# 0xEigenLabs/eigen-zeth

Hardware: AMD Instinct MI355X
Metric: goldilocks_ntt_field_elems_per_s (higher is better)
Workload: dtype u64; 1 GPU; forward NTT, natural order in/out, 2^24 rows x 64 columns per GPU (column-major u64), BASELINE configs[3] shape on one GPU; logn=24, cols_per_gpu=64, cols_total=64

## Files before the change

### eigen_zeth_amd/csrc/ntt.hip

```cpp
#include <hip/hip_runtime.h>

#include <cstring>
#include <string>

#include "ctx.hpp"
#include "wave_xchg.hpp"
#include "gl_asm.hpp"
#include "gl_limb.hpp"

#define ZP_LDG(p) __builtin_nontemporal_load(p)
#define ZP_STG(p, v) __builtin_nontemporal_store(v, p)

namespace {

typedef __attribute__((ext_vector_type(4))) int zp_i32x4;

struct PassArgs {
    const u64 *in;
    u64 *out;
    u64 in_cs, out_cs;
    u64 in_valid;
    const u64 *twl, *twh;
    const u64 *tws;
    const u64 *tw1;
    const u64 *itab;
    const u64 *csl, *csh;
    u64 scale;
    int logn, logPprev, lb, cslb;
    int j0inv;
    int logPin;
    int flags;
    int ncols;
};

__device__ __forceinline__ constexpr int brev(int x, int bits) {
    int r = 0;
    for (int i = 0; i < bits; i++) r |= ((x >> i) & 1) << (bits - 1 - i);
    return r;
}
__device__ __forceinline__ constexpr int slot_of(int o, int j, int pos, int A) {
    return ((o >> pos) << (pos + A)) | (j << pos) | (o & ((1 << pos) - 1));
}

template <int A1, int A2, int A3, int LOGT>
struct Geo {
    static constexpr int L = A1 + A2 + A3;
    static constexpr int R = 1 << L;
    static constexpr int T = 1 << LOGT;
    static constexpr int LT = LOGT;
    static constexpr int NT = (R * T) / 16;
    static constexpr int J = 1 + (A2 > 0 ? 1 : 0) + (A3 > 0 ? 1 : 0);
    static constexpr int POS1 = L - A1;
    static constexpr int POS2 = L - A1 - A2;
    static constexpr int AJ = (J == 1) ? A1 : (J == 2 ? A2 : A3);
    __device__ static __forceinline__ int kof(int sigma) {
        int k = (sigma >> POS1) & ((1 << A1) - 1);
        if (A2 > 0) k |= ((sigma >> POS2) & ((1 << A2) - 1)) << A1;
        if (A3 > 0) k |= (sigma & ((1 << A3) - 1)) << (A1 + A2);
        return k;
    }
    __device__ static __forceinline__ int sigma_of_k(int k) {
        int s = (k & ((1 << A1) - 1)) << POS1;
        if (A2 > 0) s |= ((k >> A1) & ((1 << A2) - 1)) << POS2;
        if (A3 > 0) s |= (k >> (A1 + A2)) & ((1 << A3) - 1);
        return s;
    }
    __device__ static __forceinline__ int lpos(int sigma, int t) {
        int s2 = sigma;
        if constexpr (LOGT < 4 && A3 > 0) {
            constexpr int GB = 5 - LOGT;
            s2 ^= ((sigma >> POS2) & ((1 << GB) - 1)) ^ (((sigma >> (POS1 + LOGT)) & ((1 << (A1 - LOGT)) - 1)) << 1);
        }
        return (s2 << LOGT) + (t ^ (kof(sigma) & (T - 1)));
    }
};

__device__ __forceinline__ u64 tw_lookup(const u64 *lo, const u64 *hi, int lb, u64 e) {
    u64 a = lo[e & ((1ULL << lb) - 1)];
    u64 b = hi[e >> lb];
    return gl_mul(a, b);
}

__device__ __forceinline__ u64 mul_c16(int e, u64 d) {
    switch (e) {
        case 0: return d;
        case 1: return gl_shl12<1>(d);
        case 2: return gl_shl12<2>(d);
        case 3: return gl_shl12<3>(d);
        case 4: return gl_shl12<4>(d);
        case 5: return gl_shl12<5>(d);
        case 6: return gl_shl12<6>(d);
        default: return gl_shl12<7>(d);
    }
}
template <int A>
__device__ __forceinline__ void dif_shift(u64 *v) {
    static_assert(A >= 2 && A <= 4, "radix 4, 8 or 16");
#pragma unroll
    for (int s = 0; s < A; s++) {
        const int half = 1 << (A - 1 - s);
#pragma unroll
        for (int t = 0; t < (1 << (A - 1)); t += 2) {
            const int i0 = (t / half) * 2 * half + (t % half), i1 = ((t + 1) / half) * 2 * half + ((t + 1) % half);
            gl_bfly2(v[i0], v[i0 + half], v[i1], v[i1 + half]);
            v[i0 + half] = mul_c16((t % half) * (8 / half), v[i0 + half]);
            v[i1 + half] = mul_c16(((t + 1) % half) * (8 / half), v[i1 + half]);
        }
    }
}

__device__ __forceinline__ void lds_barrier() {
    __builtin_amdgcn_fence(__ATOMIC_RELEASE, "workgroup", "local");
    __builtin_amdgcn_s_barrier();
    __builtin_amdgcn_fence(__ATOMIC_ACQUIRE, "workgroup", "local");
}

template <typename G, int ANEXT, int POSNEXT>
__device__ __forceinline__ void exchange_read(u64 *v, const u64 *lds, int tid) {
    constexpr int GN = 16 >> ANEXT;
#pragma unroll
    for (int g = 0; g < GN; g++) {
        const int gamma = g * G::NT + tid;
        const int t = gamma & (G::T - 1), o = gamma >> G::LT;
#pragma unroll
        for (int j = 0; j < (1 << ANEXT); j++)
            v[g * (1 << ANEXT) + j] = lds[G::lpos(slot_of(o, j, POSNEXT, ANEXT), t)];
    }
}

template <typename G, int A, int POS, int ANEXT, int POSNEXT, int TWSH>
__device__ __forceinline__ void exchange2(u64 *v, u64 *lds, const u64 *twr, int j0inv, int tid) {
    constexpr int GR = 16 >> A;
#pragma unroll
    for (int g = 0; g < GR; g++) {
        const int gamma = g * G::NT + tid;
        const int t = gamma & (G::T - 1), o = gamma >> G::LT;
        const int rho = o & ((1 << POS) - 1);
        {
            const int kj1 = (j0inv * brev(1, A)) & ((1 << A) - 1);
            v[g * (1 << A) + 1] = gl_mul1(v[g * (1 << A) + 1], twr[(kj1 * rho) << TWSH]);
        }
#pragma unroll
        for (int p = 2; p < (1 << A); p += 2) {
            const int kja = (j0inv * brev(p, A)) & ((1 << A) - 1), kjb = (j0inv * brev(p + 1, A)) & ((1 << A) - 1);
            gl_mul2(v[g * (1 << A) + p], twr[(kja * rho) << TWSH], v[g * (1 << A) + p + 1], twr[(kjb * rho) << TWSH]);
        }
#pragma unroll
        for (int p = 0; p < (1 << A); p++) {
            const int kj = (j0inv * brev(p, A)) & ((1 << A) - 1);
            lds[G::lpos(slot_of(o, kj, POS, A), t)] = v[g * (1 << A) + p];
        }
    }
    lds_barrier();
    exchange_read<G, ANEXT, POSNEXT>(v, lds, tid);
}

template <int E>
__device__ __forceinline__ gl_l4 mul_c16_l4(const gl_l4 &d) { return gl_l4_mul_c16<E>(d); }
__device__ __forceinline__ gl_l4 mul_c16_l4(int e, const gl_l4 &d) {
    switch (e) {
        case 0: return d;
        case 1: return gl_l4_mul_c16<1>(d);
        case 2: return gl_l4_mul_c16<2>(d);
        case 3: return gl_l4_mul_c16<3>(d);
        case 4: return gl_l4_mul_c16<4>(d);
        case 5: return gl_l4_mul_c16<5>(d);
        case 6: return gl_l4_mul_c16<6>(d);
        default: return gl_l4_mul_c16<7>(d);
    }
}
template <int A>
__device__ __forceinline__ void dif_levels_l4(gl_l4 *x) {
    static_assert(A >= 2 && A <= 4, "radix 4, 8 or 16");
#pragma unroll
    for (int s = 0; s < A; s++) {
        const int half = 1 << (A - 1 - s);
#pragma unroll
        for (int t = 0; t < (1 << (A - 1)); t++) {
            const int i0 = (t / half) * 2 * half + (t % half);
            const gl_l4 a = x[i0], b = x[i0 + half];
            x[i0] = gl_l4_add(a, b);
            x[i0 + half] = mul_c16_l4((t % half) * (8 / half), gl_l4_sub(a, b));
        }
    }
}
template <int A>
__device__ __forceinline__ void dif_shift_l4(const u64 *v, gl_l4 *x) {
#pragma unroll
    for (int i = 0; i < (1 << A); i++) x[i] = gl_l4_from(v[i]);
    dif_levels_l4<A>(x);
}
__device__ __forceinline__ gl_w4 w4_load(const gl_w4 *p) {
    const zp_i32x4 a = *(const zp_i32x4 *)p->lo, b = *(const zp_i32x4 *)p->hi;
    gl_w4 w;
    w.lo[0] = a.x; w.lo[1] = a.y; w.lo[2] = a.z; w.lo[3] = a.w;
    w.hi[0] = b.x; w.hi[1] = b.y; w.hi[2] = b.z; w.hi[3] = b.w;
    return w;
}
__device__ __forceinline__ void w4_store(gl_w4 *p, const u64 w0, const u64 w1, const u64 w2, const u64 w3) {
    i32 l[4], h[4];
    gl_l4_balance(w0, l[0], h[0]);
    gl_l4_balance(w1, l[1], h[1]);
    gl_l4_balance(w2, l[2], h[2]);
    gl_l4_balance(w3, l[3], h[3]);
    zp_i32x4 a = {l[0], l[1], l[2], l[3]}, b = {h[0], h[1], h[2], h[3]};
    *(zp_i32x4 *)p->lo = a;
    *(zp_i32x4 *)p->hi = b;
}
template <typename G, int A, int POS, int ANEXT, int POSNEXT>
__device__ __forceinline__ void exchange2_l4(const gl_l4 *x, u64 *v, u64 *lds, const gl_w4 *twr4, int j0inv, int tid) {
    constexpr int GR = 16 >> A;
#pragma unroll
    for (int g = 0; g < GR; g++) {
        const int gamma = g * G::NT + tid;
        const int t = gamma & (G::T - 1), o = gamma >> G::LT;
        const int rho = o & ((1 << POS) - 1);
#pragma unroll
        for (int p = 0; p < (1 << A); p++) {
            const int kj = (j0inv * brev(p, A)) & ((1 << A) - 1);
            const u64 y = p == 0 ? gl_l4_canon(x[g * (1 << A)]) : gl_l4_mul(x[g * (1 << A) + p], w4_load(twr4 + kj * rho));
            lds[G::lpos(slot_of(o, kj, POS, A), t)] = y;
        }
    }
    lds_barrier();
    exchange_read<G, ANEXT, POSNEXT>(v, lds, tid);
}

template <typename G>
__device__ __forceinline__ void table_copy_out(u64 *v, const u64 *lds, const u64 *twb, u64 *blk, int tid) {
    constexpr int L = G::L, NT = G::NT;
#pragma unroll
    for (int i = 0; i < 16; i++) v[i] = twb[i * NT + tid];
    lds_barrier();
#pragma unroll
    for (int i = 0; i < 16; i += 2) {
        const int ia = i * NT + tid, ib = (i + 1) * NT + tid;
        u64 xa = lds[G::lpos(G::sigma_of_k(ia & ((1 << L) - 1)), ia >> L)];
        u64 xb = lds[G::lpos(G::sigma_of_k(ib & ((1 << L) - 1)), ib >> L)];
        gl_mul2(xa, v[i], xb, v[i + 1]);
        ZP_STG(&blk[ia], xa);
        ZP_STG(&blk[ib], xb);
    }
}

template <int A1, int A2, int A3, int LOGT, bool TRANSPOSE, bool PADDED, int MODE, bool BIG = false, bool LIMB = false>
__global__ void __launch_bounds__((1 << (A1 + A2 + A3 + LOGT)) / 16, LIMB ? 3 : 4)
ntt_pass2_kernel(PassArgs a, int tiles_per_wg) {
    using G = Geo<A1, A2, A3, LOGT>;
    constexpr int L = G::L, R = G::R, T = G::T, NT = G::NT, AJ = G::AJ;
    constexpr int GRJ = 16 >> AJ;
    constexpr int R2 = 1 << (A2 + A3);
    constexpr bool HAS_TAB = !TRANSPOSE && MODE >= 1;
    constexpr bool TWR_LDS = L <= 10;
    constexpr int TPL = (R + NT - 1) / NT;
    extern __shared__ __attribute__((aligned(16))) u64 lds[];
    constexpr int REC = LIMB ? 4 : 1;
    u64 *tab = lds + R * T;
    u64 *twr1 = tab + (HAS_TAB ? R * REC : 0);
    u64 *twr2 = twr1 + R * REC;
    constexpr bool TW1 = TRANSPOSE && MODE == 3;
    constexpr bool CAN_IN = !TRANSPOSE && MODE == 0 && L <= 9;
    u64 *itl = twr2 + (TWR_LDS ? R2 * REC : 0);
    const bool in_tab = CAN_IN && a.itab != nullptr;
    static_assert(!LIMB || (TWR_LDS && (TW1 || !TRANSPOSE)), "limb form: LDS twiddle copies, no per-lane twiddle chain");
    u64 col = blockIdx.y, wg_lin = blockIdx.x;
    if constexpr (TW1) {
        const u64 x = blockIdx.x & 7u, j = blockIdx.x >> 3;
        col = j % (u64)a.ncols;
        wg_lin = (j / (u64)a.ncols) * 8 + x;
    }
    const int logNR = a.logn - L;
    const int logP = a.logPprev;
    const u64 N = 1ULL << a.logn;
    const u64 *src = a.in + col * a.in_cs;
    u64 *dst = a.out + col * a.out_cs;
    u64 v[16], vn[16];
    constexpr int NTW = TW1 ? 1 : TRANSPOSE ? (GRJ + 2) : (MODE == 2 ? TPL + 1 : TPL);
    u64 twl_c[NTW], twh_c[NTW], twl_n[NTW], twh_n[NTW];

    constexpr bool small_n = !BIG;
    auto fetch_tile = [&](u64 *r, u64 *tl, u64 *th, u64 u0, int tid) {
        constexpr int GR = 16 >> A1;
        const u64 valid_rows = a.in_valid >> logNR;
#pragma unroll
        for (int g = 0; g < GR; g++) {
            const int gamma = g * NT + tid;
            const int t = gamma & (T - 1), o = gamma >> LOGT;
            const u32 slot0 = (u32)slot_of(o, 0, G::POS1, A1);
            const u32 lane_bytes = (((u32)slot0 << logNR) + (u32)t) << 3;
            const u64 lane_el = ((u64)slot0 << logNR) + (u64)t;
#pragma unroll
            for (int j = 0; j < (1 << A1); j++) {
                const u64 *rowp = src + (((u64)j << G::POS1) << logNR) + u0;
                const u64 *ptr;
                if constexpr (small_n) ptr = (const u64 *)((const char *)rowp + lane_bytes);
                else ptr = rowp + lane_el;
                u64 val;
                if constexpr (PADDED) val = (u64)(slot0 + ((u32)j << G::POS1)) < valid_rows ? (LOGT < 4 ? *ptr : ZP_LDG(ptr)) : 0ULL;
                else val = LOGT < 4 ? *ptr : ZP_LDG(ptr);
                r[g * (1 << A1) + j] = val;
            }
        }
        const u64 lm = (1ULL << a.lb) - 1;
        if constexpr (TW1) {
            (void)tl; (void)th; (void)lm;
        } else if constexpr (TRANSPOSE) {
            const int t = tid & (T - 1);
            const u64 u = u0 + t;
            const int jr = a.j0inv & ((1 << AJ) - 1);
            u64 e[NTW];
#pragma unroll
            for (int g = 0; g < GRJ; g++) e[g] = u * (u64)G::kof(((g * NT + tid) >> LOGT) << AJ);
            e[GRJ] = ((u << (L - AJ)) * (u64)jr) & (N - 1);
            e[GRJ + 1] = (N - ((u << L) & (N - 1))) & (N - 1);
#pragma unroll
            for (int i = 0; i < NTW; i++) { tl[i] = a.twl[e[i] & lm]; th[i] = a.twh[e[i] >> a.lb]; }
        } else {
            if constexpr (MODE == 1) {
                if (a.flags & 1) {
                    const u64 e0 = (u0 >> logP) << logP;
#pragma unroll
                    for (int j = 0; j < TPL; j++) {
                        const u64 e = e0 * (u64)((tid + j * NT) & (R - 1));
                        tl[j] = a.twl[e & lm];
                        th[j] = a.twh[e >> a.lb];
                    }
                }
            }
            if constexpr (CAN_IN) {
                if (in_tab) {
                    const u64 *row = a.itab + ((u0 >> a.logPin) << L);
#pragma unroll
                    for (int j = 0; j < TPL; j++) tl[j] = row[(tid + j * NT) & (R - 1)];
                }
            }
            if constexpr (MODE == 2) {
                const u64 c = (u0 + (tid & (T - 1))) & ((1ULL << logP) - 1);
                tl[TPL] = a.csl[c & ((1ULL << a.cslb) - 1)];
                th[TPL] = a.csh[c >> a.cslb];
            }
        }
    };

    u64 wg = wg_lin;
    if constexpr (LOGT < 4 && !TW1) {
        if ((gridDim.x & 7u) == 0) wg = (u64)(blockIdx.x & 7u) * (gridDim.x >> 3) + (blockIdx.x >> 3);
    }
    const u64 tile0 = wg * tiles_per_wg;
    fetch_tile(v, twl_c, twh_c, tile0 << LOGT, threadIdx.x);
    const bool out_tab = HAS_TAB && (MODE == 2 || (a.flags & 3) != 0);
    const bool tile_tab = HAS_TAB && (a.flags & 1) != 0;
    {
        const int tid0 = threadIdx.x;
        if constexpr (LIMB) {
            for (int e = tid0; e < R; e += NT) {
                const int rot = (a.j0inv * (R / 8)) & (R - 1);
                w4_store((gl_w4 *)twr1 + e, a.tws[e << (12 - L)], a.tws[((e + rot) & (R - 1)) << (12 - L)],
                         a.tws[((e + 2 * rot) & (R - 1)) << (12 - L)], a.tws[((e + 3 * rot) & (R - 1)) << (12 - L)]);
            }
            if constexpr (G::J >= 3) {
                constexpr int L2 = A2 + A3;
                for (int e = tid0; e < R2; e += NT) {
                    const int rot = (a.j0inv * (R2 / 8)) & (R2 - 1);
                    w4_store((gl_w4 *)twr2 + e, a.tws[e << (12 - L2)], a.tws[((e + rot) & (R2 - 1)) << (12 - L2)],
                             a.tws[((e + 2 * rot) & (R2 - 1)) << (12 - L2)], a.tws[((e + 3 * rot) & (R2 - 1)) << (12 - L2)]);
                }
            }
        } else if constexpr (TWR_LDS) {
            if (tid0 < R) twr1[tid0] = a.tws[tid0 << (12 - L)];
            if constexpr (G::J >= 3) {
                if (tid0 < R2) twr2[tid0] = a.tws[tid0 << (12 - (A2 + A3))];
            }
        }
        if constexpr (HAS_TAB) {
            if (out_tab && !tile_tab) {
#pragma unroll
                for (int j = 0; j < TPL; j++)
                    if (tid0 + j * NT < R) {
                        u64 w = (a.flags & 2) ? a.scale : 1;
                        if constexpr (MODE == 2) {
                            const u64 ek = (u64)(tid0 + j * NT) << logP;
                            const u64 ck = gl_mul(a.csl[ek & ((1ULL << a.cslb) - 1)], a.csh[ek >> a.cslb]);
                            w = (a.flags & 2) ? gl_mul(w, ck) : ck;
                        }
                        if constexpr (LIMB) w4_store((gl_w4 *)tab + tid0 + j * NT, w, gl_shl12<2>(w), gl_shl12<4>(w), gl_shl12<6>(w));
                        else tab[tid0 + j * NT] = w;
                    }
            }
        }
        if constexpr (CAN_IN) {
            if (in_tab) {
#pragma unroll
                for (int j = 0; j < TPL; j++)
                    if (tid0 + j * NT < R) itl[tid0 + j * NT] = twl_c[j];
            }
        }
    }
    lds_barrier();
    __builtin_amdgcn_s_waitcnt(0x0F70);
#pragma clang loop unroll(disable)
    for (int it = 0; it < tiles_per_wg; it++) {
        const u64 u0 = (tile0 + it) << LOGT;
        const bool more = it + 1 < tiles_per_wg;
        int tid = threadIdx.x;
        asm volatile("" : "+v"(tid));
        if (more) fetch_tile(vn, twl_n, twh_n, u0 + T, tid);

        const u64 s = TRANSPOSE ? 0 : (u0 >> logP);
        if constexpr (HAS_TAB) {
            if (tile_tab) {
#pragma unroll
                for (int j = 0; j < TPL; j++)
                    if (tid + j * NT < R) {
                        const u64 w = gl_mul(twl_c[j], twh_c[j]);
                        if constexpr (LIMB) w4_store((gl_w4 *)tab + tid + j * NT, w, gl_shl12<2>(w), gl_shl12<4>(w), gl_shl12<6>(w));
                        else tab[tid + j * NT] = w;
                    }
            }
        }
        if constexpr (CAN_IN) {
            if (in_tab) {
#pragma unroll
                for (int g = 0; g < (16 >> A1); g++) {
                    const int slot0 = slot_of((g * NT + tid) >> LOGT, 0, G::POS1, A1);
#pragma unroll
                    for (int j = 0; j < (1 << A1); j += 2)
                        gl_mul2(v[g * (1 << A1) + j], itl[(j << G::POS1) + slot0], v[g * (1 << A1) + j + 1], itl[((j + 1) << G::POS1) + slot0]);
                }
            }
        }
        gl_l4 x[LIMB ? 16 : 1];
        if constexpr (LIMB) {
#pragma unroll
            for (int g = 0; g < (16 >> A1); g++) dif_shift_l4<A1>(v + g * (1 << A1), x + g * (1 << A1));
            exchange2_l4<G, A1, G::POS1, A2, G::POS2>(x, v, lds, (const gl_w4 *)twr1, a.j0inv, tid);
#pragma unroll
            for (int g = 0; g < (16 >> A2); g++) dif_shift_l4<A2>(v + g * (1 << A2), x + g * (1 << A2));
            if constexpr (G::J >= 3) {
                exchange2_l4<G, A2, G::POS2, A3, 0>(x, v, lds, (const gl_w4 *)twr2, a.j0inv, tid);
#pragma unroll
                for (int g = 0; g < (16 >> A3); g++) dif_shift_l4<A3>(v + g * (1 << A3), x + g * (1 << A3));
            }
        } else {
#pragma unroll
        for (int g = 0; g < (16 >> A1); g++) dif_shift<A1>(v + g * (1 << A1));
        exchange2<G, A1, G::POS1, A2, G::POS2, TWR_LDS ? 0 : 12 - L>(v, lds, TWR_LDS ? twr1 : a.tws, a.j0inv, tid);
#pragma unroll
        for (int g = 0; g < (16 >> A2); g++) dif_shift<A2>(v + g * (1 << A2));
        if constexpr (G::J >= 3) {
            exchange2<G, A2, G::POS2, A3, 0, TWR_LDS ? 0 : 12 - (A2 + A3)>(v, lds, TWR_LDS ? twr2 : a.tws, a.j0inv, tid);
#pragma unroll
            for (int g = 0; g < (16 >> A3); g++) dif_shift<A3>(v + g * (1 << A3));
        }
        }
#pragma unroll
        for (int g = 0; g < GRJ; g++) {
            const int gamma = g * NT + tid;
            const int t = gamma & (T - 1), o = gamma >> LOGT;
            const int klow = G::kof(o << AJ);
            if constexpr (TW1) {
                const int jr = a.j0inv & ((1 << AJ) - 1);
#pragma unroll
                for (int i = 0; i < (1 << AJ); i++) {
                    const int kj = (jr * i) & ((1 << AJ) - 1);
                    if constexpr (LIMB) lds[G::lpos(slot_of(o, kj, 0, AJ), t)] = gl_l4_canon(x[g * (1 << AJ) + brev(i, AJ)]);
                    else lds[G::lpos(slot_of(o, kj, 0, AJ), t)] = v[g * (1 << AJ) + brev(i, AJ)];
                }
            } else if constexpr (TRANSPOSE) {
                const int jr = a.j0inv & ((1 << AJ) - 1);
                u64 w = gl_mul(twl_c[g], twh_c[g]);
                const u64 hj = gl_mul(twl_c[GRJ], twh_c[GRJ]);
                const u64 hjd = gl_mul(hj, gl_mul(twl_c[GRJ + 1], twh_c[GRJ + 1]));
#pragma unroll
                for (int i = 0; i < (1 << AJ); i++) {
                    const int p = brev(i, AJ);
                    const int kj = (jr * i) & ((1 << AJ) - 1);
                    u64 x = v[g * (1 << AJ) + p];
                    if (i + 1 < (1 << AJ)) {
                        const bool wrap = ((jr * (i + 1)) >> AJ) != ((jr * i) >> AJ);
                        u64 wn = w;
                        gl_mul2(x, w, wn, wrap ? hjd : hj);
                        w = wn;
                    } else {
                        x = gl_mul1(x, w);
                    }
                    lds[G::lpos(slot_of(o, kj, 0, AJ), t)] = x;
                }
            } else {
                u64 *const sbase = dst + (s << (logP + L)) + (u0 & ((1ULL << logP) - 1));
                const u32 lane_sb = (((u32)klow << logP) + (u32)t) << 3;
                const u64 lane_se = ((u64)klow << logP) + (u64)t;
                u64 cw = 1;
                if constexpr (MODE == 2) cw = gl_mul(twl_c[TPL], twh_c[TPL]);
#pragma unroll
                for (int p = 0; p < (1 << AJ); p += 2) {
                    const int kja = (a.j0inv * brev(p, AJ)) & ((1 << AJ) - 1), kjb = (a.j0inv * brev(p + 1, AJ)) & ((1 << AJ) - 1);
                    const int ka = klow + (kja << (L - AJ)), kb = klow + (kjb << (L - AJ));
                    u64 xa, xb;
                    if constexpr (LIMB) {
                        if (out_tab) {
                            xa = gl_l4_mul(x[g * (1 << AJ) + p], w4_load((const gl_w4 *)tab + ka));
                            xb = gl_l4_mul(x[g * (1 << AJ) + p + 1], w4_load((const gl_w4 *)tab + kb));
                        } else {
                            xa = gl_l4_canon(x[g * (1 << AJ) + p]);
                            xb = gl_l4_canon(x[g * (1 << AJ) + p + 1]);
                        }
                    } else {
                        xa = v[g * (1 << AJ) + p];
                        xb = v[g * (1 << AJ) + p + 1];
                        if (out_tab) gl_mul2(xa, tab[ka], xb, tab[kb]);
                    }
                    if constexpr (MODE == 2) gl_mul2(xa, cw, xb, cw);
                    u64 *const ua = sbase + ((u64)(kja << (L - AJ)) << logP), *const ub = sbase + ((u64)(kjb << (L - AJ)) << logP);
                    u64 *pa, *pb;
                    if constexpr (small_n) { pa = (u64 *)((char *)ua + lane_sb); pb = (u64 *)((char *)ub + lane_sb); }
                    else { pa = ua + lane_se; pb = ub + lane_se; }
                    if constexpr (LOGT < 4) {
                        *pa = xa;
                        *pb = xb;
                    } else {
                        ZP_STG(pa, xa);
                        ZP_STG(pb, xb);
                    }
                }
            }
        }
        if constexpr (TW1) {
            table_copy_out<G>(v, lds, a.tw1 + (u0 << L), dst + (u0 << L), tid);
        } else if constexpr (TRANSPOSE) {
            lds_barrier();
            u64 *blk = dst + (u0 << L);
#pragma unroll
            for (int i = 0; i < 16; i++) {
                const int idx = i * NT + tid;
                const int t2 = idx >> L, k = idx & ((1 << L) - 1);
                ZP_STG(&blk[idx], lds[G::lpos(G::sigma_of_k(k), t2)]);
            }
        }
        if (more) {
            if constexpr (CAN_IN) {
                if (in_tab) {
#pragma unroll
                    for (int j = 0; j < TPL; j++)
                        if (tid + j * NT < R) itl[tid + j * NT] = twl_n[j];
                }
            }
            lds_barrier();
#pragma unroll
            for (int i = 0; i < 16; i++) v[i] = vn[i];
#pragma unroll
            for (int i = 0; i < NTW; i++) { twl_c[i] = twl_n[i]; twh_c[i] = twh_n[i]; }
        }
    }
}

struct SeamArgs {
    const u64 *in;
    u64 *out;
    u64 *coef;
    const u64 *tws_i, *tws_f;
    const u64 *tw1;
    const u64 *csl, *csh;
    u64 scale;
    int logn, cslb, j0inv_i, j0inv_f, ncols;
};
__global__ void __launch_bounds__(256, 4) lde_seam_kernel(SeamArgs a, int tiles_per_wg) {
    using G = Geo<4, 4, 0, 4>;
    constexpr int L = 8, R = 256, T = 16, LOGT = 4;
    extern __shared__ __attribute__((aligned(16))) u64 lds[];
    u64 *tab = lds + R * T;
    u64 *twr_i = tab + R;
    u64 *twr_f = twr_i + R;
    const u64 x8 = blockIdx.x & 7u, jj = blockIdx.x >> 3;
    const u64 col = jj % (u64)a.ncols, wg = (jj / (u64)a.ncols) * 8 + x8;
    const int logNR = a.logn - L;
    const u64 N = 1ULL << a.logn;
    const u64 *src = a.in + col * N;
    u64 *dst = a.out + col * (2 * N);
    u64 *cdst = a.coef ? a.coef + col * N : nullptr;
    u64 v[16];
    u64 cw_c[2];
    auto fetch_tile = [&](u64 *r, u64 *cwr, u64 u0, int tid) {
        const int t = tid & (T - 1), o = tid >> LOGT;
        const u32 slot0 = (u32)slot_of(o, 0, G::POS1, 4);
        const u32 lane_bytes = (((u32)slot0 << logNR) + (u32)t) << 3;
#pragma unroll
        for (int j = 0; j < 16; j++) {
            const u64 *rowp = src + (((u64)j << G::POS1) << logNR) + u0;
            r[j] = ZP_LDG((const u64 *)((const char *)rowp + lane_bytes));
        }
        const u64 c = u0 + (u64)t;
        cwr[0] = a.csl[c & ((1ULL << a.cslb) - 1)];
        cwr[1] = a.csh[c >> a.cslb];
    };
    const u64 tile0 = wg * tiles_per_wg;
    {
        const int tid0 = threadIdx.x;
        twr_i[tid0] = a.tws_i[tid0 << (12 - L)];
        twr_f[tid0] = a.tws_f[tid0 << (12 - L)];
        const u64 ek = (u64)tid0 << logNR;
        tab[tid0] = gl_mul(a.scale, gl_mul(a.csl[ek & ((1ULL << a.cslb) - 1)], a.csh[ek >> a.cslb]));
    }
    lds_barrier();
#pragma clang loop unroll(disable)
    for (int it = 0; it < tiles_per_wg; it++) {
        const u64 u0 = (tile0 + it) << LOGT;
        int tid = threadIdx.x;
        asm volatile("" : "+v"(tid));
        fetch_tile(v, cw_c, u0, tid);
        const int t = tid & (T - 1), o = tid >> LOGT;
        dif_shift<4>(v);
        exchange2<G, 4, G::POS1, 4, G::POS2, 0>(v, lds, twr_i, a.j0inv_i, tid);
        dif_shift<4>(v);
        const u64 cw = gl_mul(cw_c[0], cw_c[1]);
        lds_barrier();
#pragma unroll
        for (int p = 0; p < 16; p += 2) {
            const int kja = (a.j0inv_i * brev(p, 4)) & 15, kjb = (a.j0inv_i * brev(p + 1, 4)) & 15;
            const int ka = o + (kja << 4), kb = o + (kjb << 4);
            u64 xa = v[p], xb = v[p + 1];
            gl_mul2(xa, tab[ka], xb, tab[kb]);
            gl_mul2(xa, cw, xb, cw);
            if (cdst) {
                ZP_STG((u64 *)((char *)(cdst + ((u64)ka << logNR) + u0) + (t << 3)), xa);
                ZP_STG((u64 *)((char *)(cdst + ((u64)kb << logNR) + u0) + (t << 3)), xb);
            }
            lds[(((ka & 1) << 7) + (ka >> 1)) * T + t] = xa;
            lds[(((kb & 1) << 7) + (kb >> 1)) * T + t] = xb;
        }
        lds_barrier();
        u64 f1[8];
#pragma unroll
        for (int j = 0; j < 8; j++) {
            v[j] = lds[((j << 4) + o) * T + t];
            f1[j] = lds[(128 + (j << 4) + o) * T + t];
        }
        lds_barrier();
#pragma unroll 1
        for (int par = 0; par < 2; par++) {
            if (par) {
#pragma unroll
                for (int j = 0; j < 8; j++) v[j] = f1[j];
            }
#pragma unroll
            for (int j = 1; j < 8; j++) v[8 + j] = mul_c16(j, v[j]);
            v[8] = v[0];
            dif_shift<3>(v);
            dif_shift<3>(v + 8);
            exchange2<G, 4, G::POS1, 4, G::POS2, 0>(v, lds, twr_f, a.j0inv_f, tid);
            dif_shift<4>(v);
            {
                const int jr = a.j0inv_f & 15;
#pragma unroll
                for (int i = 0; i < 16; i++) {
                    const int kj = (jr * i) & 15;
                    lds[G::lpos(slot_of(o, kj, 0, 4), t)] = v[brev(i, 4)];
                }
            }
            const u64 u0f = ((u64)par << logNR) + u0;
            table_copy_out<G>(v, lds, a.tw1 + (u0f << L), dst + (u0f << L), tid);
            lds_barrier();
        }
    }
}

struct SmallArgs {
    const u64 *in;
    u64 *out;
    u64 in_cs, out_cs, in_valid;
    const u64 *tws;
    const u64 *csl, *csh;
    u64 scale;
    int logn, cslb, flags;
};

template <int LH>
__device__ __forceinline__ u64 wave_stage(u64 x, int lane, const u64 *tws) {
    const u64 y = lane_xor<LH>(x);
    const int i = lane & ((1 << LH) - 1);
    if (!((lane >> LH) & 1)) return gl_add(x, y);
    const u64 d = gl_sub(y, x);
    return i ? gl_mul(d, tws[(u64)i << (12 - (LH + 1))]) : d;
}

template <bool WAVE>
__global__ void __launch_bounds__(256) ntt_small_kernel(SmallArgs a) {
    extern __shared__ __attribute__((aligned(16))) u64 lds[];
    const int tid = threadIdx.x;
    const int n = 1 << a.logn;
    const u64 *src = a.in + (u64)blockIdx.x * a.in_cs;
    u64 *dst = a.out + (u64)blockIdx.x * a.out_cs;
    for (int i = tid; i < n; i += 256) lds[i] = (u64)i < a.in_valid ? src[i] : 0ULL;
    __syncthreads();
    const int lds_stages = WAVE ? (a.logn > 6 ? a.logn - 6 : 0) : a.logn;
    for (int s = 0; s < lds_stages; s++) {
        const int lh = a.logn - 1 - s;
        const int half = 1 << lh;
        for (int b = tid; b < (n >> 1); b += 256) {
            const int i = b & (half - 1);
            const int i0 = ((b >> lh) << (lh + 1)) + i, i1 = i0 + half;
            u64 x = lds[i0], y = lds[i1];
            lds[i0] = gl_add(x, y);
            u64 d = gl_sub(x, y);
            lds[i1] = i ? gl_mul(d, a.tws[(u64)i << (12 - (lh + 1))]) : d;
        }
        __syncthreads();
    }
    if constexpr (WAVE) {
        const int lane = tid & 63;
        for (int base = (tid >> 6) << 6; base < n; base += 256) {
            u64 x = base + lane < n ? lds[base + lane] : 0ULL;
            const int top = a.logn < 6 ? a.logn : 6;
            if (top >= 6) x = wave_stage<5>(x, lane, a.tws);
            if (top >= 5) x = wave_stage<4>(x, lane, a.tws);
            if (top >= 4) x = wave_stage<3>(x, lane, a.tws);
            if (top >= 3) x = wave_stage<2>(x, lane, a.tws);
            if (top >= 2) x = wave_stage<1>(x, lane, a.tws);
            if (top >= 1) x = wave_stage<0>(x, lane, a.tws);
            const int i = base + lane;
            if (i < n) {
                const int k = brev(i, a.logn);
                if (a.flags & 2) x = gl_mul(x, a.scale);
                if (a.flags & 4) x = gl_mul(x, tw_lookup(a.csl, a.csh, a.cslb, (u64)k));
                dst[k] = x;
            }
        }
        return;
    }
    for (int i = tid; i < n; i += 256) {
        const int k = brev(i, a.logn);
        u64 x = lds[i];
        if (a.flags & 2) x = gl_mul(x, a.scale);
        if (a.flags & 4) x = gl_mul(x, tw_lookup(a.csl, a.csh, a.cslb, (u64)k));
        dst[k] = x;
    }
}

__global__ void __launch_bounds__(256) coset_scale_kernel(const u64 *in, u64 *out, u64 n, const u64 *lo,
                                                         const u64 *hi, int lb) {
    const u64 col = blockIdx.y;
    const u64 i = ((u64)blockIdx.x * 256 + threadIdx.x);
    if (i < n) out[col * n + i] = gl_mul(in[col * n + i], tw_lookup(lo, hi, lb, i));
}

__global__ void __launch_bounds__(256) twiddle_rows_kernel(u64 *rows, int logn_row, u64 total, u64 row0, u64 nmask,
                                                           const u64 *lo, const u64 *hi, int lb) {
    const u64 i = (u64)blockIdx.x * 256 + threadIdx.x;
    if (i >= total) return;
    const u64 r = i >> logn_row, k = i & ((1ULL << logn_row) - 1);
    const u64 e = ((row0 + r) * k) & nmask;
    rows[i] = gl_mul(rows[i], tw_lookup(lo, hi, lb, e));
}

__global__ void __launch_bounds__(256) tw1_fill_kernel(u64 *out, int logn, int L, const u64 *lo, const u64 *hi, int lb) {
    const u64 i = (u64)blockIdx.x * 256 + threadIdx.x;
    if (i >> logn) return;
    const u64 u = i >> L, k = i & ((1ULL << L) - 1);
    out[i] = tw_lookup(lo, hi, lb, (u * k) & ((1ULL << logn) - 1));
}

__global__ void __launch_bounds__(256) itab_fill_kernel(u64 *out, u64 total, int logn, int L, int logPp, u64 pre, const u64 *lo, const u64 *hi, int lb) {
    const u64 i = (u64)blockIdx.x * 256 + threadIdx.x;
    if (i >= total) return;
    const u64 k = i >> L, r = i & ((1ULL << L) - 1);
    out[i] = gl_mul(pre, tw_lookup(lo, hi, lb, ((k * r) << logPp) & ((1ULL << logn) - 1)));
}

using PassKernel = void (*)(PassArgs, int);

template <int A1, int A2, int A3, int LOGT, bool BIG>
PassKernel pick_pass_kernel(bool transpose, bool table, bool padded, int mode, bool limb) {
    constexpr bool CAN_TABLE = !BIG && A3 == 0, CAN_LIMB = !BIG && A1 + A2 + A3 <= 8;
    if constexpr (CAN_TABLE) {
        if (table && limb) return padded ? ntt_pass2_kernel<A1, A2, A3, LOGT, true, true, 3, false, CAN_LIMB> : ntt_pass2_kernel<A1, A2, A3, LOGT, true, false, 3, false, CAN_LIMB>;
        if (table) return padded ? ntt_pass2_kernel<A1, A2, A3, LOGT, true, true, 3, false> : ntt_pass2_kernel<A1, A2, A3, LOGT, true, false, 3, false>;
    }
    if (transpose) return padded ? ntt_pass2_kernel<A1, A2, A3, LOGT, true, true, 1, BIG> : ntt_pass2_kernel<A1, A2, A3, LOGT, true, false, 1, BIG>;
    if (limb) return mode == 2 ? ntt_pass2_kernel<A1, A2, A3, LOGT, false, false, 2, BIG, CAN_LIMB>
                   : mode == 1 ? ntt_pass2_kernel<A1, A2, A3, LOGT, false, false, 1, BIG, CAN_LIMB>
                               : ntt_pass2_kernel<A1, A2, A3, LOGT, false, false, 0, BIG, CAN_LIMB>;
    return mode == 2 ? ntt_pass2_kernel<A1, A2, A3, LOGT, false, false, 2, BIG>
         : mode == 1 ? ntt_pass2_kernel<A1, A2, A3, LOGT, false, false, 1, BIG>
                     : ntt_pass2_kernel<A1, A2, A3, LOGT, false, false, 0, BIG>;
}

template <int A1, int A2, int A3, int LOGT, bool BIG = false>
int32_t launch_pass2(zp_ctx *ctx, PassArgs a, bool transpose, int W) {
    using G = Geo<A1, A2, A3, LOGT>;
    const u64 tiles = (1ULL << (a.logn - G::L)) >> LOGT;
    int tpw = ctx->tune_tpw;
    while (tpw > 1 && (tiles % tpw != 0 || tiles / tpw * (u64)W < (u64)ctx->num_cu * 4)) tpw >>= 1;
    dim3 grid((unsigned)(tiles / tpw), (unsigned)W), block(G::NT);
    const bool table = !BIG && A3 == 0 && transpose && a.tw1 && (grid.x & 7u) == 0;
    const int mode = transpose ? 0 : (a.flags & 4) ? 2 : (a.flags & 11) ? 1 : 0;
    const bool limb = !BIG && G::L <= 8 && ctx->tune_ntt_limb != 0 && (!transpose || table);
    const size_t rec = limb ? 4 : 1;
    const size_t shmem = ((size_t)G::R * G::T + (mode >= 1 ? G::R * rec : 0) + (G::L <= 10 ? (G::R + (1 << (A2 + A3))) * rec : 0) + (a.itab ? G::R : 0)) * sizeof(u64);
    const PassKernel k = pick_pass_kernel<A1, A2, A3, LOGT, BIG>(transpose, table, a.in_valid != (1ULL << a.logn), mode, limb);
    if (shmem > 65536) ZP_HIP(ctx, hipFuncSetAttribute((const void *)k, hipFuncAttributeMaxDynamicSharedMemorySize, (int)shmem));
    if (table) {
        a.ncols = W;
        grid = dim3(grid.x * (unsigned)W);
    }
    hipLaunchKernelGGL(k, grid, block, shmem, ctx->stream, a, tpw);
    ZP_HIP(ctx, hipGetLastError());
    return ZP_OK;
}

constexpr int shape_key(int A1, int A2, int A3, int logT, bool big) { return (((A1 * 8 + A2) * 8 + A3) * 8 + logT) * 2 + big; }

int32_t dispatch_pass(zp_ctx *ctx, const NttPass &p, const PassArgs &a, bool transpose, int W) {
    const bool big = a.logn > 28;
    const NttPassShape s = zpi_pass_shape(ctx, p.L, big, transpose, (a.flags & 7) != 0 || a.itab);
#define ZP_PASS_SHAPE(A1, A2, A3, LOGT, BIG) case shape_key(A1, A2, A3, LOGT, BIG): return launch_pass2<A1, A2, A3, LOGT, BIG>(ctx, a, transpose, W)
    switch (shape_key(s.A1, s.A2, s.A3, s.logT, big)) {
        ZP_PASS_SHAPE(3, 2, 0, 5, false);
        ZP_PASS_SHAPE(3, 3, 0, 5, false);
        ZP_PASS_SHAPE(4, 3, 0, 5, false);
        ZP_PASS_SHAPE(4, 3, 0, 5, true);
        ZP_PASS_SHAPE(4, 4, 0, 4, false);
        ZP_PASS_SHAPE(4, 4, 0, 4, true);
        ZP_PASS_SHAPE(4, 4, 0, 5, false);
        ZP_PASS_SHAPE(3, 3, 3, 4, false);
        ZP_PASS_SHAPE(3, 3, 3, 5, false);
        ZP_PASS_SHAPE(4, 3, 3, 4, false);
        ZP_PASS_SHAPE(4, 4, 3, 3, false);
        ZP_PASS_SHAPE(4, 4, 4, 1, false);
        ZP_PASS_SHAPE(4, 4, 4, 2, false);
        default: ctx->err = big ? "pass radix not built for transforms above 2^28 rows" : "unsupported pass radix"; return ZP_ERR_UNSUPPORTED;
    }
#undef ZP_PASS_SHAPE
}

struct PassTimer {
    zp_ctx *ctx;
    zp_ctx::PassEv ev;
    bool on;
    PassTimer(zp_ctx *c, int radix_log) : ctx(c), on(c->profiling) {
        ev.radix_log = radix_log;
        on = on && hipEventCreate(&ev.a) == hipSuccess && hipEventCreate(&ev.b) == hipSuccess && hipEventRecord(ev.a, ctx->stream) == hipSuccess;
    }
    ~PassTimer() {
        if (on && hipEventRecord(ev.b, ctx->stream) == hipSuccess) ctx->pass_events.push_back(ev);
    }
};

template <typename Args>
void set_output_scaling(Args &a, bool inverse, const CosetTable *post_scale) {
    if (inverse) a.flags |= 2;
    if (post_scale) {
        a.flags |= 4;
        a.csl = post_scale->d_lo;
        a.csh = post_scale->d_hi;
        a.cslb = post_scale->lb;
    }
}

int chunk_columns(const zp_ctx *ctx, int logn, int W) {
    const int wc = (int)((1ULL << (ctx->tune_ntt_chunk_log > 0 ? ctx->tune_ntt_chunk_log : 28)) >> logn);
    return wc < 1 ? 1 : wc > W ? W : wc;
}

}

NttPassShape zpi_pass_shape(const zp_ctx *ctx, int L, bool big, bool transpose, bool multiplies) {
    static const NttPassShape by_l[8] = {{3, 2, 0, 5}, {3, 3, 0, 5}, {4, 3, 0, 5}, {4, 4, 0, 4}, {3, 3, 3, 4}, {4, 3, 3, 4}, {4, 4, 3, 3}, {4, 4, 4, 2}};
    if (L < 5 || L > 12 || (big && L != 7 && L != 8)) return {0, 0, 0, 0};
    NttPassShape s = by_l[L - 5];
    if (big) return s;
    if ((L == 8 && ctx->tune_logt != 4) || (L == 9 && ctx->tune_logt9 != 4)) s.logT = 5;
    if (L == 12 && ctx->tune_logt12 == 1 && (transpose || !multiplies)) s.logT = 1;
    return s;
}

NttPassShape zpi_plan_pass_shape(const zp_ctx *ctx, const NttPlan *pl, int i) {
    return zpi_pass_shape(ctx, pl->pass[i].L, pl->logn > 28, i == 0, i + 1 < pl->npass || pl->inverse);
}

static int32_t upload_power_table(zp_ctx *ctx, int logn, u64 base, u64 pre, int *lb, u64 **d_lo, u64 **d_hi) {
    *lb = (logn + 1) / 2;
    std::vector<u64> lo(1ULL << *lb), hi(1ULL << (logn - *lb));
    lo[0] = pre;
    u64 sp = 1;
    for (size_t i = 1; i < lo.size(); i++) {
        sp = gl_mul(sp, base);
        lo[i] = gl_mul(pre, sp);
    }
    const u64 sl = gl_mul(sp, base);
    hi[0] = 1;
    for (size_t i = 1; i < hi.size(); i++) hi[i] = gl_mul(hi[i - 1], sl);
    ZP_TRY(zpi_upload(ctx, lo, d_lo));
    return zpi_upload(ctx, hi, d_hi);
}

int32_t zpi_get_plan_role(zp_ctx *ctx, int logn, bool inverse, int role, NttPlan **out) {
    const int maxl = (ctx->tune_ntt_maxl >= 6 && ctx->tune_ntt_maxl <= 12) ? ctx->tune_ntt_maxl : 9;
    const int order = ctx->tune_ntt_order;
    const int key = (((logn * 2 + (inverse ? 1 : 0)) * 16 + maxl) * 4 + (order & 3)) * 4 + (role & 3);
    int rdig[6], nr = 0;
    if (role) {
        const int r = logn - 8, m_default = (logn + maxl - 1) / maxl;
        if (logn <= 12 || r < 5 || maxl != 9) return ZP_ERR_UNSUPPORTED;
        nr = (r + maxl - 1) / maxl;
        if (1 + nr > m_default || nr > 4) return ZP_ERR_UNSUPPORTED;
        int rem = r;
        for (int i = 0; i < nr; i++) {
            int d = (rem + (nr - i) - 1) / (nr - i);
            if (i == 0 && nr >= 2 && d < 7 && rem - 7 >= 5 * (nr - 1)) d = 7;
            rdig[i] = d;
            rem -= d;
        }
        for (int i = 0; i < nr; i++)
            if (rdig[i] < 5 || rdig[i] > 9) return ZP_ERR_UNSUPPORTED;
    }
    auto it = ctx->plans.find(key);
    if (it != ctx->plans.end()) {
        *out = &it->second;
        return ZP_OK;
    }
    NttPlan pl;
    pl.logn = logn;
    pl.inverse = inverse;
    pl.role = role;
    u64 w = gl_root(ctx->root32, logn);
    u64 w4096 = gl_root(ctx->root32, 12);
    u64 w16 = gl_root(ctx->root32, 4);
    if (inverse) {
        w = gl_inv(w);
        w4096 = gl_inv(w4096);
        w16 = gl_inv(w16);
    }
    pl.ninv = gl_inv((1ULL << logn) % GL_P);
    pl.j0inv = 0;
    for (int j = 1; j < 16; j += 2)
        if (gl_pow(1ULL << 12, (u64)j) == w16)
            for (int ji = 1; ji < 16; ji += 2)
                if (((j * ji) & 15) == 1) pl.j0inv = ji;
    pl.w16[0] = 1;
    for (int i = 1; i < 8; i++) pl.w16[i] = gl_mul(pl.w16[i - 1], w16);
    std::vector<u64> tws(4096);
    tws[0] = 1;
    for (int i = 1; i < 4096; i++) tws[i] = gl_mul(tws[i - 1], w4096);
    ZP_TRY(zpi_upload(ctx, tws, &pl.d_tws));
    int dig[6];
    if (logn > 12 && role) {
        pl.npass = nr + 1;
        for (int i = 0; i < pl.npass; i++) dig[i] = role == 1 ? (i < nr ? rdig[i] : 8) : (i == 0 ? 8 : rdig[i - 1]);
    } else if (logn > 12) {
        const int m = pl.npass = (logn + maxl - 1) / maxl;
        int rem = logn, digits[6];
        for (int i = 0; i < m; i++) {
// ... 298 lines not shown
```

Measured before the change: 96.05 billion field-elems/s.

## Specialize NTT pass kernel on table mode and ping-pong tile buffers

Runtime table flags (in_tab, out_tab, tile_tab) become a compile-time template parameter, so dead branches are removed and the host picks among specialized instantiations. Row base pointers and scalar args are pinned in SGPRs through opaque asm and use global address space, which cuts VGPR address arithmetic. The tile loop is manually unrolled by two, alternating the current and next buffers so the per-tile register copy of v/vn and the twiddle arrays goes away. This adds more kernel instantiations and an unsupported-combination error path, and the asm barriers could block some compiler optimizations.

New measurement: 99.25 billion field-elems/s (median of 6 runs). +3.3%, better.

```diff
diff --git a/eigen_zeth_amd/csrc/ntt.hip b/eigen_zeth_amd/csrc/ntt.hip
--- a/eigen_zeth_amd/csrc/ntt.hip
+++ b/eigen_zeth_amd/csrc/ntt.hip
@@ -14,6 +14,24 @@
 namespace {
 
 typedef __attribute__((ext_vector_type(4))) int zp_i32x4;
+typedef __attribute__((address_space(1))) u64 zp_gu64;
+typedef __attribute__((address_space(1))) char zp_gchar;
+
+template <bool ON>
+__device__ __forceinline__ u64 sgpr_opaque(u64 x) {
+    if constexpr (!ON) return x;
+    u32 lo = (u32)x, hi = (u32)(x >> 32);
+    asm("" : "+s"(lo), "+s"(hi));
+    return ((u64)hi << 32) | lo;
+}
+template <bool ON>
+__device__ __forceinline__ int sgpr_opaque_once(int x) {
+    if constexpr (!ON) return x;
+    asm volatile("" : "+s"(x));
+    return x;
+}
+
+constexpr int TAB_NONE = 0, TAB_FIXED = 1 , TAB_TILE = 2 , TAB_IN = 3 ;
 
 struct PassArgs {
     const u64 *in;
@@ -243,7 +261,7 @@
     }
 }
 
-template <int A1, int A2, int A3, int LOGT, bool TRANSPOSE, bool PADDED, int MODE, bool BIG = false, bool LIMB = false>
+template <int A1, int A2, int A3, int LOGT, bool TRANSPOSE, bool PADDED, int MODE, int TAB, bool BIG = false, bool LIMB = false>
 __global__ void __launch_bounds__((1 << (A1 + A2 + A3 + LOGT)) / 16, LIMB ? 3 : 4)
 ntt_pass2_kernel(PassArgs a, int tiles_per_wg) {
     using G = Geo<A1, A2, A3, LOGT>;
@@ -261,7 +279,11 @@
     constexpr bool TW1 = TRANSPOSE && MODE == 3;
     constexpr bool CAN_IN = !TRANSPOSE && MODE == 0 && L <= 9;
     u64 *itl = twr2 + (TWR_LDS ? R2 * REC : 0);
-    const bool in_tab = CAN_IN && a.itab != nullptr;
+    constexpr bool LEAN = !LIMB && !(TRANSPOSE && MODE == 1);
+    constexpr bool in_tab = TAB == TAB_IN;
+    constexpr bool out_tab = TAB == TAB_FIXED || TAB == TAB_TILE;
+    constexpr bool tile_tab = TAB == TAB_TILE;
+    static_assert((!in_tab || CAN_IN) && (!out_tab || (HAS_TAB && (MODE == 1 || !tile_tab))) && (MODE != 2 || out_tab), "a table the pass has no place for");
     static_assert(!LIMB || (TWR_LDS && (TW1 || !TRANSPOSE)), "limb form: LDS twiddle copies, no per-lane twiddle chain");
     u64 col = blockIdx.y, wg_lin = blockIdx.x;
     if constexpr (TW1) {
@@ -279,7 +301,7 @@
     u64 twl_c[NTW], twh_c[NTW], twl_n[NTW], twh_n[NTW];
 
     constexpr bool small_n = !BIG;
-    auto fetch_tile = [&](u64 *r, u64 *tl, u64 *th, u64 u0, int tid) {
+    auto fetch_tile = [&](u64 *r, u64 *tl, u64 *th, u64 u0, int tid) __attribute__((always_inline)) {
         constexpr int GR = 16 >> A1;
         const u64 valid_rows = a.in_valid >> logNR;
 #pragma unroll
@@ -289,11 +311,13 @@
             const u32 slot0 = (u32)slot_of(o, 0, G::POS1, A1);
             const u32 lane_bytes = (((u32)slot0 << logNR) + (u32)t) << 3;
             const u64 lane_el = ((u64)slot0 << logNR) + (u64)t;
+            u64 row_at = sgpr_opaque<LEAN>((u64)(src + u0));
 #pragma unroll
             for (int j = 0; j < (1 << A1); j++) {
-                const u64 *rowp = src + (((u64)j << G::POS1) << logNR) + u0;
-                const u64 *ptr;
-                if constexpr (small_n) ptr = (const u64 *)((const char *)rowp + lane_bytes);
+                const zp_gu64 *rowp = (const zp_gu64 *)row_at;
+                row_at = sgpr_opaque<LEAN>(row_at + ((8ULL << G::POS1) << logNR));
+                const zp_gu64 *ptr;
+                if constexpr (small_n) ptr = (const zp_gu64 *)((const zp_gchar *)rowp + lane_bytes);
                 else ptr = rowp + lane_el;
                 u64 val;
                 if constexpr (PADDED) val = (u64)(slot0 + ((u32)j << G::POS1)) < valid_rows ? (LOGT < 4 ? *ptr : ZP_LDG(ptr)) : 0ULL;
@@ -317,7 +341,7 @@
             for (int i = 0; i < NTW; i++) { tl[i] = a.twl[e[i] & lm]; th[i] = a.twh[e[i] >> a.lb]; }
         } else {
             if constexpr (MODE == 1) {
-                if (a.flags & 1) {
+                if constexpr (tile_tab) {
                     const u64 e0 = (u0 >> logP) << logP;
 #pragma unroll
                     for (int j = 0; j < TPL; j++) {
@@ -328,7 +352,7 @@
                 }
             }
             if constexpr (CAN_IN) {
-                if (in_tab) {
+                if constexpr (in_tab) {
                     const u64 *row = a.itab + ((u0 >> a.logPin) << L);
 #pragma unroll
                     for (int j = 0; j < TPL; j++) tl[j] = row[(tid + j * NT) & (R - 1)];
@@ -348,8 +372,6 @@
     }
     const u64 tile0 = wg * tiles_per_wg;
     fetch_tile(v, twl_c, twh_c, tile0 << LOGT, threadIdx.x);
-    const bool out_tab = HAS_TAB && (MODE == 2 || (a.flags & 3) != 0);
-    const bool tile_tab = HAS_TAB && (a.flags & 1) != 0;
     {
         const int tid0 = threadIdx.x;
         if constexpr (LIMB) {
@@ -373,7 +395,7 @@
             }
         }
         if constexpr (HAS_TAB) {
-            if (out_tab && !tile_tab) {
+            if constexpr (TAB == TAB_FIXED) {
 #pragma unroll
                 for (int j = 0; j < TPL; j++)
                     if (tid0 + j * NT < R) {
@@ -389,7 +411,7 @@
             }
         }
         if constexpr (CAN_IN) {
-            if (in_tab) {
+            if constexpr (in_tab) {
 #pragma unroll
                 for (int j = 0; j < TPL; j++)
                     if (tid0 + j * NT < R) itl[tid0 + j * NT] = twl_c[j];
@@ -398,17 +420,18 @@
     }
     lds_barrier();
     __builtin_amdgcn_s_waitcnt(0x0F70);
-#pragma clang loop unroll(disable)
-    for (int it = 0; it < tiles_per_wg; it++) {
+    auto tile_step = [&](u64 *v, u64 *twl_c, u64 *twh_c, u64 *vn, u64 *twl_n, u64 *twh_n, int it) __attribute__((always_inline)) {
         const u64 u0 = (tile0 + it) << LOGT;
         const bool more = it + 1 < tiles_per_wg;
         int tid = threadIdx.x;
         asm volatile("" : "+v"(tid));
+        const int j0inv = sgpr_opaque_once<LEAN>(a.j0inv);
+        const int logP = sgpr_opaque_once<LEAN>(a.logPprev);
         if (more) fetch_tile(vn, twl_n, twh_n, u0 + T, tid);
 
         const u64 s = TRANSPOSE ? 0 : (u0 >> logP);
         if constexpr (HAS_TAB) {
-            if (tile_tab) {
+            if constexpr (tile_tab) {
 #pragma unroll
                 for (int j = 0; j < TPL; j++)
                     if (tid + j * NT < R) {
@@ -419,7 +442,7 @@
             }
         }
         if constexpr (CAN_IN) {
-            if (in_tab) {
+            if constexpr (in_tab) {
 #pragma unroll
                 for (int g = 0; g < (16 >> A1); g++) {
                     const int slot0 = slot_of((g * NT + tid) >> LOGT, 0, G::POS1, A1);
@@ -433,22 +456,22 @@
         if constexpr (LIMB) {
 #pragma unroll
             for (int g = 0; g < (16 >> A1); g++) dif_shift_l4<A1>(v + g * (1 << A1), x + g * (1 << A1));
-            exchange2_l4<G, A1, G::POS1, A2, G::POS2>(x, v, lds, (const gl_w4 *)twr1, a.j0inv, tid);
+            exchange2_l4<G, A1, G::POS1, A2, G::POS2>(x, v, lds, (const gl_w4 *)twr1, j0inv, tid);
 #pragma unroll
             for (int g = 0; g < (16 >> A2); g++) dif_shift_l4<A2>(v + g * (1 << A2), x + g * (1 << A2));
             if constexpr (G::J >= 3) {
-                exchange2_l4<G, A2, G::POS2, A3, 0>(x, v, lds, (const gl_w4 *)twr2, a.j0inv, tid);
+                exchange2_l4<G, A2, G::POS2, A3, 0>(x, v, lds, (const gl_w4 *)twr2, j0inv, tid);
 #pragma unroll
                 for (int g = 0; g < (16 >> A3); g++) dif_shift_l4<A3>(v + g * (1 << A3), x + g * (1 << A3));
             }
         } else {
 #pragma unroll
         for (int g = 0; g < (16 >> A1); g++) dif_shift<A1>(v + g * (1 << A1));
-        exchange2<G, A1, G::POS1, A2, G::POS2, TWR_LDS ? 0 : 12 - L>(v, lds, TWR_LDS ? twr1 : a.tws, a.j0inv, tid);
+        exchange2<G, A1, G::POS1, A2, G::POS2, TWR_LDS ? 0 : 12 - L>(v, lds, TWR_LDS ? twr1 : a.tws, j0inv, tid);
 #pragma unroll
         for (int g = 0; g < (16 >> A2); g++) dif_shift<A2>(v + g * (1 << A2));
         if constexpr (G::J >= 3) {
-            exchange2<G, A2, G::POS2, A3, 0, TWR_LDS ? 0 : 12 - (A2 + A3)>(v, lds, TWR_LDS ? twr2 : a.tws, a.j0inv, tid);
+            exchange2<G, A2, G::POS2, A3, 0, TWR_LDS ? 0 : 12 - (A2 + A3)>(v, lds, TWR_LDS ? twr2 : a.tws, j0inv, tid);
 #pragma unroll
             for (int g = 0; g < (16 >> A3); g++) dif_shift<A3>(v + g * (1 << A3));
         }
@@ -459,7 +482,7 @@
             const int t = gamma & (T - 1), o = gamma >> LOGT;
             const int klow = G::kof(o << AJ);
             if constexpr (TW1) {
-                const int jr = a.j0inv & ((1 << AJ) - 1);
+                const int jr = j0inv & ((1 << AJ) - 1);
 #pragma unroll
                 for (int i = 0; i < (1 << AJ); i++) {
                     const int kj = (jr * i) & ((1 << AJ) - 1);
@@ -467,7 +490,7 @@
                     else lds[G::lpos(slot_of(o, kj, 0, AJ), t)] = v[g * (1 << AJ) + brev(i, AJ)];
                 }
             } else if constexpr (TRANSPOSE) {
-                const int jr = a.j0inv & ((1 << AJ) - 1);
+                const int jr = j0inv & ((1 << AJ) - 1);
                 u64 w = gl_mul(twl_c[g], twh_c[g]);
                 const u64 hj = gl_mul(twl_c[GRJ], twh_c[GRJ]);
                 const u64 hjd = gl_mul(hj, gl_mul(twl_c[GRJ + 1], twh_c[GRJ + 1]));
@@ -494,11 +517,11 @@
                 if constexpr (MODE == 2) cw = gl_mul(twl_c[TPL], twh_c[TPL]);
 #pragma unroll
                 for (int p = 0; p < (1 << AJ); p += 2) {
-                    const int kja = (a.j0inv * brev(p, AJ)) & ((1 << AJ) - 1), kjb = (a.j0inv * brev(p + 1, AJ)) & ((1 << AJ) - 1);
+                    const int kja = (j0inv * brev(p, AJ)) & ((1 << AJ) - 1), kjb = (j0inv * brev(p + 1, AJ)) & ((1 << AJ) - 1);
                     const int ka = klow + (kja << (L - AJ)), kb = klow + (kjb << (L - AJ));
                     u64 xa, xb;
                     if constexpr (LIMB) {
-                        if (out_tab) {
+                        if constexpr (out_tab) {
                             xa = gl_l4_mul(x[g * (1 << AJ) + p], w4_load((const gl_w4 *)tab + ka));
                             xb = gl_l4_mul(x[g * (1 << AJ) + p + 1], w4_load((const gl_w4 *)tab + kb));
                         } else {
@@ -508,12 +531,13 @@
                     } else {
                         xa = v[g * (1 << AJ) + p];
                         xb = v[g * (1 << AJ) + p + 1];
-                        if (out_tab) gl_mul2(xa, tab[ka], xb, tab[kb]);
+                        if constexpr (out_tab) gl_mul2(xa, tab[ka], xb, tab[kb]);
                     }
                     if constexpr (MODE == 2) gl_mul2(xa, cw, xb, cw);
-                    u64 *const ua = sbase + ((u64)(kja << (L - AJ)) << logP), *const ub = sbase + ((u64)(kjb << (L - AJ)) << logP);
-                    u64 *pa, *pb;
-                    if constexpr (small_n) { pa = (u64 *)((char *)ua + lane_sb); pb = (u64 *)((char *)ub + lane_sb); }
+                    zp_gu64 *const ua = (zp_gu64 *)sgpr_opaque<LEAN>((u64)(sbase + ((u64)(kja << (L - AJ)) << logP)));
+                    zp_gu64 *const ub = (zp_gu64 *)sgpr_opaque<LEAN>((u64)(sbase + ((u64)(kjb << (L - AJ)) << logP)));
+                    zp_gu64 *pa, *pb;
+                    if constexpr (small_n) { pa = (zp_gu64 *)((zp_gchar *)ua + lane_sb); pb = (zp_gu64 *)((zp_gchar *)ub + lane_sb); }
                     else { pa = ua + lane_se; pb = ub + lane_se; }
                     if constexpr (LOGT < 4) {
                         *pa = xa;
@@ -539,20 +563,37 @@
         }
         if (more) {
             if constexpr (CAN_IN) {
-                if (in_tab) {
+                if constexpr (in_tab) {
 #pragma unroll
                     for (int j = 0; j < TPL; j++)
                         if (tid + j * NT < R) itl[tid + j * NT] = twl_n[j];
                 }
             }
             lds_barrier();
-#pragma unroll
-            for (int i = 0; i < 16; i++) v[i] = vn[i];
-#pragma unroll
-            for (int i = 0; i < NTW; i++) { twl_c[i] = twl_n[i]; twh_c[i] = twh_n[i]; }
-        }
-    }
-}
+        }
+    };
+    if constexpr (!LEAN) {
+#pragma clang loop unroll(disable)
+        for (int it = 0; it < tiles_per_wg; it++) {
+            tile_step(v, twl_c, twh_c, vn, twl_n, twh_n, it);
+            if (it + 1 < tiles_per_wg) {
+#pragma unroll
+                for (int i = 0; i < 16; i++) v[i] = vn[i];
+#pragma unroll
+                for (int i = 0; i < NTW; i++) { twl_c[i] = twl_n[i]; twh_c[i] = twh_n[i]; }
+            }
+        }
+    } else {
+#pragma clang loop unroll(disable)
+        for (int it = 0;; it += 2) {
+            tile_step(v, twl_c, twh_c, vn, twl_n, twh_n, it);
+            if (it + 1 >= tiles_per_wg) break;
+            tile_step(vn, twl_n, twh_n, v, twl_c, twh_c, it + 1);
+            if (it + 2 >= tiles_per_wg) break;
+        }
+    }
+}
+
 
 struct SeamArgs {
     const u64 *in;
@@ -768,20 +809,28 @@
 
 using PassKernel = void (*)(PassArgs, int);
 
+template <int A1, int A2, int A3, int LOGT, bool BIG, bool LIMB>
+PassKernel pick_later_pass(int mode, int tab) {
+    if (mode == 2) return tab == TAB_FIXED ? ntt_pass2_kernel<A1, A2, A3, LOGT, false, false, 2, TAB_FIXED, BIG, LIMB> : nullptr;
+    if (mode == 1)
+        return tab == TAB_TILE    ? ntt_pass2_kernel<A1, A2, A3, LOGT, false, false, 1, TAB_TILE, BIG, LIMB>
+               : tab == TAB_FIXED ? ntt_pass2_kernel<A1, A2, A3, LOGT, false, false, 1, TAB_FIXED, BIG, LIMB>
+               : tab == TAB_NONE  ? ntt_pass2_kernel<A1, A2, A3, LOGT, false, false, 1, TAB_NONE, BIG, LIMB>
+                                  : nullptr;
+    if constexpr (A1 + A2 + A3 <= 9) {
+        if (tab == TAB_IN) return ntt_pass2_kernel<A1, A2, A3, LOGT, false, false, 0, TAB_IN, BIG, LIMB>;
+    }
+    return tab == TAB_NONE ? ntt_pass2_kernel<A1, A2, A3, LOGT, false, false, 0, TAB_NONE, BIG, LIMB> : nullptr;
+}
 template <int A1, int A2, int A3, int LOGT, bool BIG>
-PassKernel pick_pass_kernel(bool transpose, bool table, bool padded, int mode, bool limb) {
+PassKernel pick_pass_kernel(bool transpose, bool table, bool padded, int mode, int tab, bool limb) {
     constexpr bool CAN_TABLE = !BIG && A3 == 0, CAN_LIMB = !BIG && A1 + A2 + A3 <= 8;
     if constexpr (CAN_TABLE) {
-        if (table && limb) return padded ? ntt_pass2_kernel<A1, A2, A3, LOGT, true, true, 3, false, CAN_LIMB> : ntt_pass2_kernel<A1, A2, A3, LOGT, true, false, 3, false, CAN_LIMB>;
-        if (table) return padded ? ntt_pass2_kernel<A1, A2, A3, LOGT, true, true, 3, false> : ntt_pass2_kernel<A1, A2, A3, LOGT, true, false, 3, false>;
-    }
-    if (transpose) return padded ? ntt_pass2_kernel<A1, A2, A3, LOGT, true, true, 1, BIG> : ntt_pass2_kernel<A1, A2, A3, LOGT, true, false, 1, BIG>;
-    if (limb) return mode == 2 ? ntt_pass2_kernel<A1, A2, A3, LOGT, false, false, 2, BIG, CAN_LIMB>
-                   : mode == 1 ? ntt_pass2_kernel<A1, A2, A3, LOGT, false, false, 1, BIG, CAN_LIMB>
-                               : ntt_pass2_kernel<A1, A2, A3, LOGT, false, false, 0, BIG, CAN_LIMB>;
-    return mode == 2 ? ntt_pass2_kernel<A1, A2, A3, LOGT, false, false, 2, BIG>
-         : mode == 1 ? ntt_pass2_kernel<A1, A2, A3, LOGT, false, false, 1, BIG>
-                     : ntt_pass2_kernel<A1, A2, A3, LOGT, false, false, 0, BIG>;
+        if (table && limb) return padded ? ntt_pass2_kernel<A1, A2, A3, LOGT, true, true, 3, TAB_NONE, false, CAN_LIMB> : ntt_pass2_kernel<A1, A2, A3, LOGT, true, false, 3, TAB_NONE, false, CAN_LIMB>;
+        if (table) return padded ? ntt_pass2_kernel<A1, A2, A3, LOGT, true, true, 3, TAB_NONE, false> : ntt_pass2_kernel<A1, A2, A3, LOGT, true, false, 3, TAB_NONE, false>;
+    }
+    if (transpose) return padded ? ntt_pass2_kernel<A1, A2, A3, LOGT, true, true, 1, TAB_NONE, BIG> : ntt_pass2_kernel<A1, A2, A3, LOGT, true, false, 1, TAB_NONE, BIG>;
+    return limb ? pick_later_pass<A1, A2, A3, LOGT, BIG, CAN_LIMB>(mode, tab) : pick_later_pass<A1, A2, A3, LOGT, BIG, false>(mode, tab);
 }
 
 template <int A1, int A2, int A3, int LOGT, bool BIG = false>
@@ -796,7 +845,12 @@
     const bool limb = !BIG && G::L <= 8 && ctx->tune_ntt_limb != 0 && (!transpose || table);
     const size_t rec = limb ? 4 : 1;
     const size_t shmem = ((size_t)G::R * G::T + (mode >= 1 ? G::R * rec : 0) + (G::L <= 10 ? (G::R + (1 << (A2 + A3))) * rec : 0) + (a.itab ? G::R : 0)) * sizeof(u64);
-    const PassKernel k = pick_pass_kernel<A1, A2, A3, LOGT, BIG>(transpose, table, a.in_valid != (1ULL << a.logn), mode, limb);
+    const int tab = transpose ? TAB_NONE : a.itab ? TAB_IN : (a.flags & 1) ? TAB_TILE : (a.flags & 6) ? TAB_FIXED : TAB_NONE;
+    const PassKernel k = pick_pass_kernel<A1, A2, A3, LOGT, BIG>(transpose, table, a.in_valid != (1ULL << a.logn), mode, tab, limb);
+    if (!k) {
+        ctx->err = "pass kernel not built for this combination of output scaling and tables";
+        return ZP_ERR_UNSUPPORTED;
+    }
     if (shmem > 65536) ZP_HIP(ctx, hipFuncSetAttribute((const void *)k, hipFuncAttributeMaxDynamicSharedMemorySize, (int)shmem));
     if (table) {
         a.ncols = W;
```
